# pjmikkol/bwtc

Hardware: AMD Instinct MI355X
Metric: MB/s compressed (BWT+encode) on 256 MiB block (higher is better)
Workload: dtype u8/u32/u64 integer

## Files before the change

### bwtc_amd/csrc/bwt_engine.hip

```cpp
#include "bwt_engine.hpp"
#include "radix_sort.hpp"
#include <algorithm>
#include <cmath>
#include <cstdlib>
#include <cstring>
#include <chrono>
#include <ctime>
#include <sys/prctl.h>

namespace bwtc_hip {

constexpr int kLoadTPB = 256;
constexpr int kLoadTile = kLoadTPB * 16;
constexpr u32 kTextPad = 128;

__global__ __launch_bounds__(kLoadTPB) void k_load_hist(const u8* __restrict__ src,
                                                        u8* __restrict__ T, u32 ncopy,
                                                        u32 padded, int reverse, int aligned,
                                                        u32* __restrict__ freqs) {
  __shared__ __attribute__((aligned(16))) u8 s_src[kLoadTile + 48];
  __shared__ u32 s_hist[256 * 16];
  const u32 tid = threadIdx.x;
  for (u32 i = tid; i < 256 * 16; i += kLoadTPB) s_hist[i] = 0;
  const u32 ntiles = (padded + (u32)kLoadTile - 1u) / (u32)kLoadTile;
// ... 1675 lines not shown
    if (std::getenv("BWTC_HIP_FIN_GROUP")) fin_max_group = std::atoi(std::getenv("BWTC_HIP_FIN_GROUP"));
    if (std::getenv("BWTC_HIP_FIN_WINDOW")) fin_window = std::atoi(std::getenv("BWTC_HIP_FIN_WINDOW"));
    fin_shape_fixed = std::getenv("BWTC_HIP_FIN_GROUP") || std::getenv("BWTC_HIP_FIN_WINDOW");
    fin_wide_short = !(std::getenv("BWTC_HIP_FIN_WIDE") && std::getenv("BWTC_HIP_FIN_WIDE")[0] == '0');
    fin_window = fin_window >= 2048 ? 2048 : 1024;
    fin_max_group = fin_max_group >= 1024 ? 1024 : fin_max_group >= 512 ? 512 : 256;
    if (fin_max_group >= fin_window) fin_max_group = fin_window / 2;
    code_keys = !(std::getenv("BWTC_HIP_KEYS") && std::strcmp(std::getenv("BWTC_HIP_KEYS"), "grams") == 0);
    if (std::getenv("BWTC_HIP_CODE_BITS")) code_bits = std::min(72, std::max(40, std::atoi(std::getenv("BWTC_HIP_CODE_BITS"))));
    finisher = !(std::getenv("BWTC_HIP_FINISHER") && std::getenv("BWTC_HIP_FINISHER")[0] == '0');
    gm_partition_lines = std::getenv("BWTC_HIP_GM_PARTITION") && std::strcmp(std::getenv("BWTC_HIP_GM_PARTITION"), "lines") == 0;
    wt_segmented = !(std::getenv("BWTC_HIP_SEG_STEPS") && std::getenv("BWTC_HIP_SEG_STEPS")[0] == '0');
    gram_min_n = kGramMinN;
    if (std::getenv("BWTC_HIP_GRAM_MIN_N")) gram_min_n = (u32)std::max(64, std::atoi(std::getenv("BWTC_HIP_GRAM_MIN_N")));
    if (std::getenv("BWTC_HIP_LONG_E")) long_items_per_thread = std::atoi(std::getenv("BWTC_HIP_LONG_E")) == 6 ? 6 : 8;
    if (std::getenv("BWTC_HIP_FIN_PASSES")) fin_max_passes = std::max(0, std::atoi(std::getenv("BWTC_HIP_FIN_PASSES")));
    if (std::getenv("BWTC_HIP_FIN_WORDS")) fin_words = std::min(4, std::max(2, std::atoi(std::getenv("BWTC_HIP_FIN_WORDS"))));
    if (std::getenv("BWTC_HIP_LONG_DIRECT")) long_direct = std::getenv("BWTC_HIP_LONG_DIRECT")[0] != '0';
    if (std::getenv("BWTC_HIP_FIN_ROUNDS")) fin_rounds = std::min(4, std::max(1, std::atoi(std::getenv("BWTC_HIP_FIN_ROUNDS"))));
    run_ranks = !(std::getenv("BWTC_HIP_RUNS") && std::getenv("BWTC_HIP_RUNS")[0] == '0');
    local_rounds = !(std::getenv("BWTC_HIP_LOCAL_ROUNDS") && std::getenv("BWTC_HIP_LOCAL_ROUNDS")[0] == '0');
    if (std::getenv("BWTC_HIP_FIN_FLOOR")) fin_floor = (u32)std::max(0, std::atoi(std::getenv("BWTC_HIP_FIN_FLOOR")));
    if (std::getenv("BWTC_HIP_TEXT_ROUNDS")) { text_rounds = std::max(0, std::atoi(std::getenv("BWTC_HIP_TEXT_ROUNDS"))); text_rounds_fixed = true; }
    const char* hg = std::getenv("BWTC_HIP_HUGE_MI");
    if (hg && std::atoi(hg) > 0) huge_group_elements = (u64)std::atoi(hg) << 20;
  }
  if (std::getenv("BWTC_HIP_SCAN") && std::strcmp(std::getenv("BWTC_HIP_SCAN"), "chained") == 0) {
    scan_chain.cap_tiles = (u32)(cap / kScanTile + 4096);
    BWTC_HIP_TRY(hipMalloc(reinterpret_cast<void**>(&scan_chain.status), ((u64)scan_chain.cap_tiles + 1) * 8));
    BWTC_HIP_TRY(hipMemset(scan_chain.status, 0, ((u64)scan_chain.cap_tiles + 1) * 8));
    scan_chain.ticket = scan_chain.status + scan_chain.cap_tiles;
    scan_chain.err = d_small + 522;
    scan_chain.stream = stream;
    scan_chain.issued = 0;
    scan_chain.epoch = 0;
  }
  BWTC_HIP_TRY(hipHostMalloc(reinterpret_cast<void**>(&h_small), 1024 * 4, hipHostMallocDefault));
  BWTC_HIP_TRY(hipHostMalloc(reinterpret_cast<void**>(&h_stage), cap + 32, hipHostMallocDefault));
  BWTC_HIP_TRY(hipEventCreateWithFlags(&ev_wait, hipEventBlockingSync | hipEventDisableTiming));
  {
    const char* m = std::getenv("BWTC_HIP_SYNC");
    wait_mode = m && std::strcmp(m, "spin") == 0 ? 1 : m && std::strcmp(m, "block") == 0 ? 2 : 0;
  }
  BWTC_HIP_TRY(hipEventCreate(&ev_begin));
  BWTC_HIP_TRY(hipEventCreate(&ev_end));
  for (int i = 0; i < kMaxSortEvents; ++i) BWTC_HIP_TRY(hipEventCreate(&ev_sort[i]));
// ... 530 lines not shown
        if (rc) return rc;
        w_bits = gp.b * lk.G2;
        if (w_bits < kRadixBits) { lk.first_r = w_bits; lk.first_mask = (1u << std::min(kRadixBits, w_bits + key_bits)) - 1u; }
        short_len = (u32)(gp.g * (gp.G + lk.G2));
        h = (u64)short_len;
        hipLaunchKernelGGL(k_make_keys_gram, dim3(ceil_div(n, 1024)), dim3(256), 0, st, d_T, d_lut,
                           (const uint4*)d_rank, ka, (u32*)nullptr, n, gp.g, gp.G, gp.b, plan.sigma, gp.top, key_plane, split, lk);
        lg.hi_shift = lk.hi_shift; lg.chr_shift = lk.chr_shift; lg.chr_mask = lk.chr_mask; lg.lvl_shift = -1; lg.depth = short_len;
        if (std::getenv("BWTC_HIP_DEBUG"))
          std::fprintf(stderr, "long keys: %d + %d bits, %d + %d grams of %d characters, character code at bit %d\n",
                       key_bits, w_bits, gp.G, lk.G2, gp.g, lk.chr_shift);
      }
    }
    if (lk.w) {
      u64* ks = nullptr; unsigned short* vs16 = nullptr; u32* ws = nullptr;
      u32* vs32 = nullptr;
      if (!split_now)
        radix_sort_long<u32, 6>(ka, kb, d_V0, d_V1, d_W0, d_W1, n, key_bits, w_bits, d_table, d_partial, stream, &ks, &vs32, &ws, &probe, d_P0, d_P1, 0, false, long_direct);
      else if (long_items_per_thread == 6)
        radix_sort_long<unsigned short, 6>(ka, kb, reinterpret_cast<unsigned short*>(d_V0), reinterpret_cast<unsigned short*>(d_V1),
                                           d_W0, d_W1, n, key_bits, w_bits, d_table, d_partial, stream, &ks, &vs16, &ws, &probe, d_P0, d_P1, 0, false, long_direct);
      else
        radix_sort_long<unsigned short, 8>(ka, kb, reinterpret_cast<unsigned short*>(d_V0), reinterpret_cast<unsigned short*>(d_V1),
                                           d_W0, d_W1, n, key_bits, w_bits, d_table, d_partial, stream, &ks, &vs16, &ws, &probe, d_P0, d_P1, 0, false, long_direct);
      BWTC_HIP_TRY(hipEventRecord(ev_sort[n_sort_events++], st));
      u32* vs = split_now ? reinterpret_cast<u32*>(vs16) : vs32;
      rb.rec_keys = ks; rb.rec_free = ks == ka ? kb : ka;
      rb.v_keys = vs; rb.v_free = vs == d_V0 ? d_V1 : d_V0;
      lg.w = ws; lg.wmask = w_bits >= 32 ? ~0u : (1u << w_bits) - 1u;
      rc = rank_step<u64, true>(ks, vs, n, n, short_len, (1ull << key_bits) - 1ull, rb, re, emit, h, &res, (u32)split_now, &lg);
      if (rc == -3 && coded && (h_small[kSmallError] & 2u)) {
        if (std::getenv("BWTC_HIP_DEBUG")) std::fprintf(stderr, "code keys: a codeword above %u bits, the block takes gram keys\n", kCodeMaxLen);
        BWTC_HIP_TRY(hipMemsetAsync(d_small + kSmallError, 0, 4, st));
        code_failed = true;
        rc = suffix_sort(n, hist, lone_sentinel, em);
        code_failed = false;
        return rc;
      }
      if (rc) return rc;
      const int long_passes = (key_bits + w_bits + kRadixBits - 1) / kRadixBits;
      stats.sort_pass_items += (u64)n * (u64)long_passes;
      stats.alg_bytes += (u64)n * (1 + 12 + 1)
                         + sort_bytes(n, long_passes, split_now ? 14 : 16, 8, true);
      stats.route |= coded ? 17u : 1u;
      key_bits = 0;
    } else if (gp.G > 0) {
      hipLaunchKernelGGL(k_make_keys_gram, dim3(ceil_div(n, 1024)), dim3(256), 0, st, d_T, d_lut,
// ... 549 lines not shown
```

### bwtc_amd/csrc/bwt_engine.hpp

```cpp
#pragma once
#include "common.hpp"
#include "bwtc_hip.h"
#include "radix_sort.hpp"
#include "scan.hpp"
#include "wavelet_host.hpp"
#include "wavelet_pipeline.hpp"
#include <sys/mman.h>
#include <condition_variable>
#include <future>
#include <map>
#include <mutex>
#include <thread>
#include <memory>
#include <utility>
#include <cstdlib>
#include <functional>
#include <vector>

namespace bwtc_hip {

struct RrEmit;
struct RrLong;
struct FinList;
struct FinShallow;
// ... 307 lines not shown
  int suffix_sort(u32 n, const u32* hist, bool lone_sentinel, const EmitTarget* em = nullptr);
  template <typename K>
  void sort_pairs(K* k0, K* k1, u32* v0, u32* v1, u64 n, int nbits, K** ks, u32** vs,
                  bool probe_it, int bit_lo = 0, u64 n_holes = 0, bool plane_ready = false, bool values_descend = false);
  struct RankBuffers { void* rec_keys; void* rec_free; u32* v_keys; u32* v_free; u32* aglob; u32* aglob_next; };
  struct RankResult { u32 m, groups; u64* ks; u32* vs; void* rec_other; u32* v_other; bool finish; u32 text_chars; bool carry;
                      bool ran_run; };
  template <typename K, bool INIT>
  int rank_step(const K* ks, const u32* vs, u32 m, u32 n, u32 short_len, K kmask, RankBuffers& rb,
                struct RrEmit re, bool emit, u64 h_next, RankResult* res, u32 split = 0,
                const struct RrLong* lg = nullptr, bool text = false, bool carry_in = true, bool raw_out = false,
                int run_mode = 0);
  bool dense_route = true;
  bool digit_planes = true;
  int window_bits = 16;
  bool split_index = true;
  bool gram_keys = true;
  int gram_count_override = 0;
  struct GramPlan { int g = 0, G = 0, b = 0; u32 top = 0; };
  int plan_grams(const KeyPlan& plan, u32 n, const u8* d_lut, GramPlan* gp);
  bool no_emit = false;
  bool long_keys = true;
  int long_items_per_thread = 8;
  u32 gram_min_n = 1u << 22;
  bool code_failed = false;
  bool code_keys = true;
  int code_bits = 72;
  u32* d_pairs = nullptr;
  u32* d_codes = nullptr;
  u32* d_parkS = nullptr;
  u64* d_parkHP = nullptr;
  u32 parked = 0;
  u32 park_holes = 0;
  u32* d_hardS = nullptr;
  u64* d_hardHP = nullptr;
  unsigned short* d_hardC = nullptr;
  bool ranks_live = false;
  u32 fin_floor = 12;
  bool finisher = true;
  int fin_window = 1024;
  int fin_max_group = 256;
  int fin_words = 2;
  bool fin_shape_fixed = false;
  bool fin_wide_short = true;
  int fin_window_blk = 1024;
  int fin_group_blk = 256;
// ... 72 lines not shown
```

### bwtc_amd/csrc/c_abi.hip

```cpp
#include "bwt_engine.hpp"
#include "gpu_lanes.hpp"
#include "huffman_decoder.hpp"
#include "postprocess.hpp"
#include "wavelet_rebuild.hpp"
#include "prepr_host.hpp"
#include <new>
#include "radix_sort.hpp"
#include "bwtc_hip.h"
#include "entropy_host.hpp"
#include "wavelet_host.hpp"
#include "wavelet_gpu_models.hpp"
#include <sched.h>
#include <algorithm>
#include <atomic>
#include <string>
#include <cstring>
#include <new>
#include <thread>
#include <vector>

using namespace bwtc_hip;

struct bwtc_hip_ctx {
  BwtEngine eng;
// ... 131 lines not shown
  V* v1 = reinterpret_cast<V*>(e.d_V1);
  std::vector<u8> plane(n);
  if (wbits >= kRadixBits) {
    for (u64 i = 0; i < n; ++i) plane[i] = (u8)(w[i] & 255u);
  } else {
    const u32 dmask = (1u << std::min(kRadixBits, wbits + kbits)) - 1u;
    for (u64 i = 0; i < n; ++i) plane[i] = (u8)((w[i] | ((u32)keys[i] << wbits)) & dmask);
  }
  SortCanaries can;
  BWTC_HIP_TRY(hipMemcpyAsync(k0, keys, n * 8, hipMemcpyHostToDevice, st));
  BWTC_HIP_TRY(hipMemcpyAsync(e.d_W0, w, n * 4, hipMemcpyHostToDevice, st));
  BWTC_HIP_TRY(hipMemcpyAsync(e.d_P0, plane.data(), n, hipMemcpyHostToDevice, st));
  BWTC_HIP_TRY(hipMemsetAsync(v0, 0xA5, n * sizeof(V), st));
  BWTC_HIP_TRY(can.put(k0, n * 8, st));
  BWTC_HIP_TRY(can.put(k1, n * 8, st));
  BWTC_HIP_TRY(can.put(v0, n * sizeof(V), st));
  BWTC_HIP_TRY(can.put(v1, n * sizeof(V), st));
  BWTC_HIP_TRY(can.put(e.d_W0, n * 4, st));
  BWTC_HIP_TRY(can.put(e.d_W1, n * 4, st));
  BWTC_HIP_TRY(can.put(e.d_P0, n, st));
  BWTC_HIP_TRY(can.put(e.d_P1, n, st));
  u64* ks = nullptr; V* vs = nullptr; u32* ws = nullptr;
  radix_sort_long<V, EL>(k0, k1, v0, v1, e.d_W0, e.d_W1, n, kbits, wbits, e.d_table, e.d_partial, st, &ks, &vs, &ws, nullptr,
                         e.d_P0, e.d_P1, 0, false, direct_w);
  BWTC_HIP_TRY(hipMemcpyAsync(keys, ks, n * 8, hipMemcpyDeviceToHost, st));
  BWTC_HIP_TRY(hipMemcpyAsync(vals, vs, n * sizeof(V), hipMemcpyDeviceToHost, st));
  BWTC_HIP_TRY(hipMemcpyAsync(w, ws, n * 4, hipMemcpyDeviceToHost, st));
  BWTC_HIP_TRY(can.fetch(st));
  BWTC_HIP_TRY(e.wait());
  BWTC_HIP_TRY(hipGetLastError());
  return can.verdict();
}
}

static std::mutex& host_allocs_mu() { static std::mutex m; return m; }
static std::map<void*, std::pair<int, uint64_t> >& host_allocs() { static std::map<void*, std::pair<int, uint64_t> > m; return m; }

static __global__ __launch_bounds__(256) void k_copy_probe(const uint4* __restrict__ src, uint4* __restrict__ dst, uint64_t n16) {
  const uint64_t i = (uint64_t)blockIdx.x * 256u + threadIdx.x;
  if (i < n16) dst[i] = src[i];
}

extern "C" {

int bwtc_hip_device_count(void) {
  int n = 0;
  if (hipGetDeviceCount(&n) != hipSuccess) return 0;
// ... 877 lines not shown

int bwtc_hip_test_radix_pairs(bwtc_hip_ctx* ctx, void* keys, void* vals, uint64_t n, uint64_t n_holes, int key_bytes, int val_bytes,
                              int bit_lo, int nbits, int values_mode, int planes) {
  if (!ctx || !keys) return -1;
  BwtEngine& e = ctx->eng;
  typedef unsigned short u16v;
  if (key_bytes == 4 && val_bytes == 4) return test_radix_pairs<u32, u32>(e, static_cast<u32*>(keys), static_cast<u32*>(vals), n, n_holes, bit_lo, nbits, values_mode, planes);
  if (key_bytes == 8 && val_bytes == 4) return test_radix_pairs<u64, u32>(e, static_cast<u64*>(keys), static_cast<u32*>(vals), n, n_holes, bit_lo, nbits, values_mode, planes);
  if (key_bytes == 4 && val_bytes == 2) return test_radix_pairs<u32, u16v>(e, static_cast<u32*>(keys), static_cast<u16v*>(vals), n, n_holes, bit_lo, nbits, values_mode, planes);
  if (key_bytes == 8 && val_bytes == 2) return test_radix_pairs<u64, u16v>(e, static_cast<u64*>(keys), static_cast<u16v*>(vals), n, n_holes, bit_lo, nbits, values_mode, planes);
  return -1;
}

int bwtc_hip_test_radix_long(bwtc_hip_ctx* ctx, uint64_t* keys, void* vals, uint32_t* w, uint64_t n, int val_bytes, int items_per_thread,
                             int kbits, int wbits, int direct_w) {
  if (!ctx || !keys || !vals || !w) return -1;
  BwtEngine& e = ctx->eng;
  typedef unsigned short u16v;
  if (val_bytes == 4 && items_per_thread == 6) return test_radix_long<u32, 6>(e, keys, static_cast<u32*>(vals), w, n, kbits, wbits, direct_w != 0);
  if (val_bytes == 2 && items_per_thread == 6) return test_radix_long<u16v, 6>(e, keys, static_cast<u16v*>(vals), w, n, kbits, wbits, direct_w != 0);
  if (val_bytes == 2 && items_per_thread == 8) return test_radix_long<u16v, 8>(e, keys, static_cast<u16v*>(vals), w, n, kbits, wbits, direct_w != 0);
  return -1;
}

int bwtc_hip_test_radix_segmented(bwtc_hip_ctx* ctx, uint32_t* keys, uint64_t n, int bit_lo, const uint32_t* tile_first, uint32_t nseg) {
  if (!ctx || !keys || !tile_first) return -1;
  BwtEngine& e = ctx->eng;
  const u64 tile = (u64)radix_tile<u32>();
  if (n == 0 || n % tile != 0 || n + kSortCanaryBytes > e.cap) return -1;
  if (bit_lo < 0 || bit_lo + 2 * kRadixBits > 32) return -1;
  if (nseg == 0 || (u64)nseg + 1 > e.cap || tile_first[0] != 0 || (u64)tile_first[nseg] != n / tile) return -1;
  for (u32 s = 0; s < nseg; ++s) if (tile_first[s] > tile_first[s + 1]) return -1;
  BWTC_HIP_TRY(hipSetDevice(e.device));
  hipStream_t st = e.stream;
  u32* k0 = static_cast<u32*>(e.d_R1);
  u32* k1 = static_cast<u32*>(e.d_R2);
  std::vector<u8> plane(n);
  for (u64 i = 0; i < n; ++i) plane[i] = (u8)((keys[i] >> bit_lo) & 255u);
  SortCanaries can;
  BWTC_HIP_TRY(hipMemcpyAsync(k0, keys, n * 4, hipMemcpyHostToDevice, st));
  BWTC_HIP_TRY(hipMemcpyAsync(e.d_P0, plane.data(), n, hipMemcpyHostToDevice, st));
  BWTC_HIP_TRY(hipMemcpyAsync(e.d_V0, tile_first, ((u64)nseg + 1) * 4, hipMemcpyHostToDevice, st));
  BWTC_HIP_TRY(can.put(k0, n * 4, st));
  BWTC_HIP_TRY(can.put(k1, n * 4, st));
  BWTC_HIP_TRY(can.put(e.d_P0, n, st));
  BWTC_HIP_TRY(can.put(e.d_P1, n, st));
// ... 217 lines not shown
```

### bwtc_amd/csrc/radix_sort.hpp

```cpp
#pragma once
#include "common.hpp"
#include "scan.hpp"
#include <algorithm>

namespace bwtc_hip {

constexpr int kRadixBits = 8;
constexpr int kRadixBins = 1 << kRadixBits;
#ifndef BWTC_RADIX_TPB
#define BWTC_RADIX_TPB 512
#endif
#ifndef BWTC_RADIX_E64
#define BWTC_RADIX_E64 8
#endif
#ifndef BWTC_RADIX_E32
#define BWTC_RADIX_E32 16
#endif
#ifndef BWTC_HIST_COPIES
#define BWTC_HIST_COPIES 16
#endif
constexpr int kRadixTPB = BWTC_RADIX_TPB;
constexpr int kRadixWaves = kRadixTPB / kWave;

#ifdef BWTC_RADIX_CHECKED
// ... 217 lines not shown
    kk[e] = i < tile_out ? s_key[i] : (K)0;
    vv[e] = (i < tile_out && !KEYS) ? s_val[i] : 0u;
    if (LONG) ww[LONG ? e : 0] = i < tile_out ? s_w[i] : 0u;
  }
#pragma unroll
  for (int e = 0; e < E; ++e)
    dst[e] = s_gofs[long_digit<K, LONG>(kk[e], ww[LONG ? e : 0], shift, la.dmask, la.bridge)] + tid + (u32)e * kRadixTPB;
#pragma unroll
  for (int e = 0; e < E; ++e) {
#ifdef BWTC_RADIX_CHECKED
    if (tid + (u32)e * kRadixTPB < tile_out && (u64)dst[e] >= n) { atomicOr(&g_radix_fault, 1u); continue; }
#endif
    if (tid + (u32)e * kRadixTPB < tile_out) {
      kout[dst[e]] = kk[e];
      if (!KEYS) vout[dst[e]] = (V)vv[e];
      if (LONG) la.wout[dst[e]] = ww[LONG ? e : 0];
      if (PLANE) {
        if (LONG) plane[dst[e]] = (u8)((la.nfrom_w == 2 ? (ww[LONG ? e : 0] >> la.nshift) | ((u32)kk[e] << la.nbridge)
                                         : la.nfrom_w ? ww[LONG ? e : 0] >> la.nshift : (u32)(kk[e] >> la.nshift)) & la.ndmask);
        else plane[dst[e]] = (u8)radix_digit(kk[e], shift + kRadixBits);
      }
    }
  }
}

template <typename K, int E_ = RadixCfg<K>::E, bool SEG = false>
__global__ __launch_bounds__(kRadixTPB) void k_radix_hist_plane(const u8* __restrict__ plane,
                                                                u32* __restrict__ table, u64 n,
                                                                u32 ntiles, SegArgs sa) {
  constexpr int E = E_;
  constexpr int HALF = kRadixTPB / 2;
  constexpr int B = 2 * E;
  static_assert(B == 8 || B == 12 || B % 16 == 0, "8-byte, 12-byte or whole 16-byte loads");
  constexpr u32 C = BWTC_HIST_COPIES;
  __shared__ __attribute__((aligned(16))) u32 hist[2][kRadixBins * C];
  {
    uint4* z = reinterpret_cast<uint4*>(&hist[0][0]);
    for (u32 i = threadIdx.x; i < 2u * kRadixBins * C / 4u; i += kRadixTPB) z[i] = make_uint4(0, 0, 0, 0);
  }
  __syncthreads();
  const u32 half = threadIdx.x / HALF, t = threadIdx.x % HALF;
  const u32 npairs = (ntiles + 1u) / 2u, per_xcd = (npairs + 7u) / 8u;
  const u32 pair = (blockIdx.x & 7u) * per_xcd + (blockIdx.x >> 3);
  const u32 tile = pair * 2u + half;
  if (pair < npairs && tile < ntiles) {
    const u64 base = (u64)tile * (kRadixTPB * E) + (u64)t * B;
// ... 167 lines not shown

static inline void radix_sort_keys_segmented(u32* k0, u32* k1, u64 n, int bit_lo, const u32* tile_first, u32 nseg,
                                             u32* table, u32* partial, hipStream_t st, u32** k_sorted,
                                             u8* plane0, u8* plane1) {
  constexpr int E = RadixCfg<u32>::E;
  const u32 ntiles = (u32)(n / radix_tile<u32>());
  const dim3 sgrid(((ntiles + 7u) / 8u) * 8u), hgrid(hist_plane_grid(ntiles)), tpb(kRadixTPB);
  SegArgs sa; sa.tile_first = tile_first; sa.nseg = nseg;
  hipLaunchKernelGGL((k_radix_hist_plane<u32, E, true>), hgrid, tpb, 0, st, (const u8*)plane0, table, n, ntiles, sa);
  exclusive_scan_u32(table, (u64)ntiles * kRadixBins, partial, st);
  hipLaunchKernelGGL((k_radix_scatter<u32, false, true, true, u32, 0, E, true>), sgrid, tpb, 0, st, (const u32*)k0, (const u32*)nullptr, k1,
                     (u32*)nullptr, (const u32*)table, n, bit_lo, ntiles, 2, plane1, LongArgs(), sa);
  hipLaunchKernelGGL((k_radix_hist_plane<u32, E, true>), hgrid, tpb, 0, st, (const u8*)plane1, table, n, ntiles, sa);
  exclusive_scan_u32(table, (u64)ntiles * kRadixBins, partial, st);
  hipLaunchKernelGGL((k_radix_scatter<u32, false, false, true, u32, 0, E, true>), sgrid, tpb, 0, st, (const u32*)k1, (const u32*)nullptr, k0,
                     (u32*)nullptr, (const u32*)table, n, bit_lo + kRadixBits, ntiles, 2, (u8*)nullptr, LongArgs(), sa);
  *k_sorted = k0;
}

template <typename V, int EL = 8>
static inline void radix_sort_long(u64* k0, u64* k1, V* v0, V* v1, u32* w0, u32* w1, u64 n, int kbits, int wbits,
                                   u32* table, u32* partial, hipStream_t st, u64** k_sorted, V** v_sorted,
                                   u32** w_sorted, ScatterProbe* probe, u8* plane0, u8* plane1, int wlo = 0,
                                   bool values_given = false, bool direct_w = true) {
  u64 *kin = k0, *kout = k1;
  V *vin = v0, *vout = v1;
  u32 *win = w0, *wout = w1;
  struct Pass { int from_w, shift; u32 dmask; int bridge; };
  Pass ps[24];
  int np = 0;
  int s = 0;
  for (; s + kRadixBits <= wbits; s += kRadixBits) ps[np++] = Pass{1, wlo + s, (1u << kRadixBits) - 1u, 0};
  int ks = 0;
  if (s < wbits) {
    const int r = wbits - s;
    ps[np++] = Pass{2, wlo + s, (1u << std::min(kRadixBits, r + kbits)) - 1u, r};
    ks = std::min(kbits, kRadixBits - r);
  }
  for (; ks < kbits; ks += kRadixBits) ps[np++] = Pass{0, ks, (1u << std::min(kRadixBits, kbits - ks)) - 1u, 0};
  if (n > 1) {
    const u32 ntiles = ceil_div(n, (u64)kRadixTPB * EL);
    const dim3 sgrid(((ntiles + 7u) / 8u) * 8u);
    for (int p = 0; p < np; ++p) {
      const bool from_words = direct_w && p > 0 && ps[p].from_w == 1 && ps[p].dmask == (1u << kRadixBits) - 1u;
      if (from_words) hipLaunchKernelGGL((k_radix_hist_words<EL>), dim3(hist_plane_grid(ntiles)), dim3(kRadixTPB), 0, st, (const u32*)win, table, n, ps[p].shift, ntiles);
      else hipLaunchKernelGGL((k_radix_hist_plane<u64, EL>), dim3(hist_plane_grid(ntiles)), dim3(kRadixTPB), 0, st, (const u8*)plane0, table, n, ntiles, SegArgs());
      exclusive_scan_u32(table, (u64)ntiles * kRadixBins, partial, st);
      const bool last = p + 1 == np;
      const bool no_plane = last || (direct_w && ps[p + 1].from_w == 1 && ps[p + 1].dmask == (1u << kRadixBits) - 1u);
      LongArgs la;
      la.win = win; la.wout = wout; la.dmask = ps[p].dmask; la.bridge = ps[p].bridge;
      la.nshift = last ? 0 : ps[p + 1].shift; la.nfrom_w = last ? 0 : ps[p + 1].from_w; la.ndmask = last ? 0u : ps[p + 1].dmask;
      la.nbridge = last ? 0 : ps[p + 1].bridge;
      const int vmode = (p == 0 && !values_given) ? 3 : 0;
      const bool timed = probe && probe->begin(st);
#define BWTC_SCATTER_L(P, L) hipLaunchKernelGGL((k_radix_scatter<u64, false, P, false, V, L, EL>), sgrid, dim3(kRadixTPB), 0, st, kin, vin, kout, vout, table, n, ps[p].shift, ntiles, vmode, no_plane ? (u8*)nullptr : plane1, la, SegArgs())
      if (ps[p].from_w == 2) { if (no_plane) BWTC_SCATTER_L(false, 3); else BWTC_SCATTER_L(true, 3); }
      else if (ps[p].from_w) { if (no_plane) BWTC_SCATTER_L(false, 2); else BWTC_SCATTER_L(true, 2); }
      else { if (no_plane) BWTC_SCATTER_L(false, 1); else BWTC_SCATTER_L(true, 1); }
#undef BWTC_SCATTER_L
      if (timed) probe->end(st, 2 * n * (sizeof(u64) + sizeof(V) + sizeof(u32)) + (no_plane ? 0 : n));
      { u8* tp = plane0; plane0 = plane1; plane1 = tp; }
      { u64* t = kin; kin = kout; kout = t; }
      { V* t = vin; vin = vout; vout = t; }
      { u32* t = win; win = wout; wout = t; }
    }
  }
  *k_sorted = kin; *v_sorted = vin; *w_sorted = win;
}


constexpr int kChains = 1;
constexpr int kSweepMaxPasses = 8;
constexpr u32 kStAgg = 1u << 30, kStIncl = 2u << 30, kStErr = 3u << 30, kStMask = (1u << 30) - 1u;
constexpr u32 kSweepSpinLimit = 1u << 22;

struct SweepWs {
  u32* hist_all;
  u32* bases;
  u32* tickets;
  u32* status;
  u32* error;
// ... 236 lines not shown
```

### bwtc_amd/hip.py

```python
import ctypes
import os

import numpy as np

_HERE = os.path.dirname(os.path.abspath(__file__))
LIB_PATH = os.environ.get("BWTC_HIP_LIB") or os.path.join(_HERE, "lib", "libbwtc_hip.so")

_vp = ctypes.c_void_p
_u32 = ctypes.c_uint32
_u64 = ctypes.c_uint64


class BwtcHipError(RuntimeError):
    def __init__(self, msg, code=None):
        super().__init__(msg)
        self.code = code


E_NO_CODE, E_SHAPE, E_PAST_RECORD, E_RUNS, E_CAPACITY, E_LENGTH = -10, -11, -12, -13, -14, -15


class HuffmanDecodeStats(ctypes.Structure):
    _fields_ = [("route", _u32), ("sections", _u32), ("streams", _u32), ("host_syncs", _u32),
                ("retries", _u32), ("max_code_len", _u32), ("runs", _u64), ("tiles", _u64), ("map_entries", _u64),
# ... 140 lines not shown
REJECT_FLAGS, REJECT_COUNT, REJECT_SCAN, REJECT_STATE, REJECT_TEST = 1, 2, 4, 8, 16


class KernelTimers(ctypes.Structure):
    _fields_ = [("scatter_launches", _u64), ("scatter_bytes", _u64), ("scatter_ms", ctypes.c_double)]


EXPORTS = [
    "bwtc_hip_huffman_decode", "bwtc_hip_huffman_decode_device", "bwtc_hip_huffman_decode_stats_get",
    "bwtc_hip_device_count", "bwtc_hip_version", "bwtc_hip_workspace_bytes", "bwtc_hip_create",
    "bwtc_hip_destroy", "bwtc_hip_stream", "bwtc_hip_get_stats", "bwtc_hip_set_profiling",
    "bwtc_hip_get_kernel_timers", "bwtc_hip_copy_probe", "bwtc_hip_test_gpu_lanes", "bwtc_hip_malloc", "bwtc_hip_free", "bwtc_hip_memcpy_to_device",
    "bwtc_hip_memcpy_to_host", "bwtc_hip_host_alloc", "bwtc_hip_host_free",
    "bwtc_hip_memcpy_to_device_async", "bwtc_hip_copy_wait", "bwtc_hip_wavelet_host_clock", "bwtc_hip_wavelet_host_progress", "bwtc_hip_wavelet_latency", "bwtc_hip_wavelet_routes", "bwtc_hip_host_staging_bytes", "bwtc_hip_host_usable_cpus", "bwtc_hip_n_lf", "bwtc_hip_bwt",
    "bwtc_hip_bwt_block", "bwtc_hip_bwt_block_device", "bwtc_hip_inverse_bwt_block",
    "bwtc_hip_inverse_bwt_block_device", "bwtc_hip_compress_bound",
    "bwtc_hip_huffman_encode_device", "bwtc_hip_huffman_encode", "bwtc_hip_transform_and_encode",
    "bwtc_hip_wavelet_section_stats", "bwtc_hip_transform_and_encode_wavelet", "bwtc_hip_wavelet_encode",
    "bwtc_hip_wavelet_encode_device", "bwtc_hip_wavelet_encode_device_begin", "bwtc_hip_wavelet_encode_end",
    "bwtc_hip_wavelet_encode_device_prepare", "bwtc_hip_wavelet_encode_queue",
    "bwtc_hip_wavelet_depth", "bwtc_hip_wavelet_set_depth", "bwtc_hip_numa_node", "bwtc_hip_host_cpu_slice", "bwtc_hip_set_worker_cpus", "bwtc_hip_wavelet_reset", "bwtc_hip_wavelet_start", "bwtc_hip_host_wavelet_sections", "bwtc_hip_host_wavelet_streams", "bwtc_hip_host_wavelet_streams_lanes", "bwtc_hip_host_huffman_lengths", "bwtc_hip_host_huffman_codes", "bwtc_hip_host_serialize_shape",
    "bwtc_hip_host_sections", "bwtc_hip_host_bwtblock_header", "bwtc_hip_synth", "bwtc_hip_suffix_array",
    "bwtc_hip_test_sort_u32", "bwtc_hip_test_sort_u64", "bwtc_hip_test_scan_u32",
    "bwtc_hip_test_radix_pairs", "bwtc_hip_test_radix_long", "bwtc_hip_test_radix_segmented",
    "bwtc_hip_wavelet_depth_needed", "bwtc_hip_grammar_create", "bwtc_hip_grammar_destroy", "bwtc_hip_grammar_rules", "bwtc_hip_grammar_special_symbols",
    "bwtc_hip_grammar_is_special", "bwtc_hip_grammar_write", "bwtc_hip_grammar_read", "bwtc_hip_pair_replace_device",
    "bwtc_hip_test_pair_stats", "bwtc_hip_precompress", "bwtc_hip_host_precompress", "bwtc_hip_postprocess",
    "bwtc_hip_postprocess_device", "bwtc_hip_postprocess_block", "bwtc_hip_postprocess_stats_get",
    "bwtc_hip_host_postprocess_tiles",
    "bwtc_hip_wavelet_decoder_create", "bwtc_hip_wavelet_decoder_destroy", "bwtc_hip_wavelet_decoder_reset",
    "bwtc_hip_wavelet_decode_bwt_host",
    "bwtc_hip_wavelet_decode_counts", "bwtc_hip_wavelet_decoder_forest", "bwtc_hip_wavelet_rebuild", "bwtc_hip_wavelet_rebuild_device",
    "bwtc_hip_host_wavelet_rebuild", "bwtc_hip_wavelet_decode_stats_get",
]

_lib = None


def load():
    global _lib
    if _lib is not None:
        return _lib
    if not os.path.exists(LIB_PATH):
        raise BwtcHipError(
            "%s not found: build it with `make -C bwtc_amd/csrc` (or __graft_entry__.build()); "
            "there is no CPU fallback" % LIB_PATH)
    L = ctypes.CDLL(LIB_PATH)
# ... 690 lines not shown
        n = keys.size - n_holes
        mode = self.RADIX_VALUES[values]
        if mode == 0:
            vals = np.array(vals, dtype=vtype, copy=True)
            assert vals.size == keys.size
        elif mode != 2:
            vals = np.zeros(max(n, 1), vtype)
        else:
            vals = None
        nbits = 8 * keys.itemsize if nbits is None else nbits
        _check(self.lib.bwtc_hip_test_radix_pairs(self.handle, _ptr(keys), None if vals is None else _ptr(vals), n, n_holes, keys.itemsize,
                                                  vtype.itemsize, bit_lo, nbits, mode, planes), "bwtc_hip_test_radix_pairs")
        return keys[:n], (None if vals is None else vals[:n])

    def test_radix_long(self, keys, w, kbits, wbits, vtype=np.uint32, items_per_thread=6, direct_w=True):
        keys = np.array(keys, dtype=np.uint64, copy=True)
        w = np.array(w, dtype=np.uint32, copy=True)
        assert keys.size == w.size
        vals = np.zeros(max(keys.size, 1), np.dtype(vtype))
        _check(self.lib.bwtc_hip_test_radix_long(self.handle, _ptr(keys), _ptr(vals), _ptr(w), keys.size, vals.itemsize, items_per_thread,
                                                 kbits, wbits, 1 if direct_w else 0), "bwtc_hip_test_radix_long")
        return keys, vals[:keys.size], w

    def test_radix_segmented(self, keys, bit_lo, tile_first):
        keys = np.array(keys, dtype=np.uint32, copy=True)
        tf = np.array(tile_first, dtype=np.uint32, copy=True)
        assert tf.size >= 2
        _check(self.lib.bwtc_hip_test_radix_segmented(self.handle, _ptr(keys), keys.size, bit_lo, _ptr(tf), tf.size - 1),
               "bwtc_hip_test_radix_segmented")
        return keys


def host_cpu_slice(numa_node, rank, ranks):
    L = load()
    buf = np.zeros(4096, np.uint32)
    n = L.bwtc_hip_host_cpu_slice(int(numa_node), int(rank), int(ranks), _ptr(buf), buf.size)
    if n < 0:
        raise BwtcHipError("bwtc_hip_host_cpu_slice failed with code %d" % n)
    return [int(c) for c in buf[:n]]


def host_staging_bytes():
    L = load()
    a, b = ctypes.c_uint64(0), ctypes.c_uint64(0)
    L.bwtc_hip_host_staging_bytes(ctypes.byref(a), ctypes.byref(b))
    return a.value, b.value
# ... 6 lines not shown
```

### include/bwtc_hip.h

```cpp
#ifndef BWTC_HIP_H
#define BWTC_HIP_H
#include <stddef.h>
#include <stdint.h>

#ifdef __cplusplus
extern "C" {
#endif

typedef struct bwtc_hip_ctx bwtc_hip_ctx;

typedef struct bwtc_hip_stats {
  uint32_t n;
  uint32_t rounds;
  uint64_t active_sum;
  uint64_t sort_pass_items;
  float    ms_total;
  float    ms_sort;
  uint32_t route;
  uint32_t finisher_entries;
  uint64_t alg_bytes;
} bwtc_hip_stats;

typedef struct bwtc_hip_kernel_timers {
  uint64_t scatter_launches;
// ... 161 lines not shown
                                  const uint8_t* run_sym, const uint32_t* run_start,
                                  const uint32_t* run_freqs, const uint32_t* dist_offset,
                                  const uint32_t* dist_len, const uint32_t* dist_cnt,
                                  uint32_t threads, char coder, uint32_t* state, uint8_t* out,
                                  uint64_t out_cap, uint64_t* out_bytes);

void     bwtc_hip_host_huffman_lengths(const uint64_t* freqs, uint8_t* clen);
void     bwtc_hip_host_huffman_codes(const uint8_t* clen, uint32_t* code);
uint32_t bwtc_hip_host_serialize_shape(const uint8_t* clen, uint8_t* out, uint32_t cap);
uint32_t bwtc_hip_host_sections(const uint32_t* freqs, uint32_t* section_len);
uint32_t bwtc_hip_host_bwtblock_header(const uint32_t* lf, uint32_t n_lf, uint8_t* out, uint32_t cap);

int bwtc_hip_synth(char kind, uint64_t seed, uint64_t size, uint8_t* out);

int bwtc_hip_suffix_array(bwtc_hip_ctx* ctx, const uint8_t* T, uint32_t length, uint32_t* sa);

int bwtc_hip_test_sort_u32(bwtc_hip_ctx* ctx, uint32_t* keys, uint32_t* vals, uint64_t n, int nbits);
int bwtc_hip_test_sort_u64(bwtc_hip_ctx* ctx, uint64_t* keys, uint32_t* vals, uint64_t n, int nbits);
int bwtc_hip_test_scan_u32(bwtc_hip_ctx* ctx, uint32_t* data, uint64_t n);
int bwtc_hip_test_radix_pairs(bwtc_hip_ctx* ctx, void* keys, void* vals, uint64_t n, uint64_t n_holes, int key_bytes, int val_bytes,
                              int bit_lo, int nbits, int values_mode, int planes);
int bwtc_hip_test_radix_long(bwtc_hip_ctx* ctx, uint64_t* keys, void* vals, uint32_t* w, uint64_t n, int val_bytes, int items_per_thread,
                             int kbits, int wbits, int direct_w);
int bwtc_hip_test_radix_segmented(bwtc_hip_ctx* ctx, uint32_t* keys, uint64_t n, int bit_lo, const uint32_t* tile_first, uint32_t nseg);
int bwtc_hip_test_gpu_lanes(bwtc_hip_ctx* ctx, const uint16_t* w, uint64_t n, const uint64_t* bounds, uint32_t k, int mode,
                            uint8_t* out, uint64_t out_cap, uint64_t* offsets);

typedef struct bwtc_hip_grammar bwtc_hip_grammar;
bwtc_hip_grammar* bwtc_hip_grammar_create(void);
void     bwtc_hip_grammar_destroy(bwtc_hip_grammar* g);
uint32_t bwtc_hip_grammar_rules(const bwtc_hip_grammar* g);
uint32_t bwtc_hip_grammar_special_symbols(const bwtc_hip_grammar* g);
int      bwtc_hip_grammar_is_special(const bwtc_hip_grammar* g, unsigned symbol);
int      bwtc_hip_grammar_write(const bwtc_hip_grammar* g, uint8_t* out, uint64_t cap, uint64_t* bytes);
int      bwtc_hip_grammar_read(bwtc_hip_grammar* g, const uint8_t* in, uint64_t n, uint64_t* consumed);
int      bwtc_hip_pair_replace_device(bwtc_hip_ctx* ctx, bwtc_hip_grammar* g, const uint8_t* d_src, uint64_t n,
                                      uint8_t* d_dst, uint64_t* n_out, uint32_t* replaced);
int      bwtc_hip_test_pair_stats(bwtc_hip_ctx* ctx, const uint8_t* d_src, uint64_t n, uint32_t* pair_cnt, uint32_t* byte_cnt);
int      bwtc_hip_precompress(bwtc_hip_ctx* ctx, bwtc_hip_grammar* g, const char* options, uint8_t* block, uint64_t n,
                              uint64_t* n_out);
int      bwtc_hip_host_precompress(bwtc_hip_grammar* g, const char* options, uint8_t* block, uint64_t n, uint64_t* n_out);
int      bwtc_hip_postprocess(const bwtc_hip_grammar* g, const uint8_t* data, uint64_t n, uint8_t* out, uint64_t cap,
                              uint64_t* n_out);
int      bwtc_hip_postprocess_device(bwtc_hip_ctx* ctx, const bwtc_hip_grammar* g, const uint8_t* d_data, uint64_t n,
                                     uint8_t* d_out, uint64_t cap, uint64_t* n_out);
int      bwtc_hip_postprocess_block(bwtc_hip_ctx* ctx, const bwtc_hip_grammar* g, const uint8_t* data, uint64_t n,
// ... 106 lines not shown
```

Measured before the change: 7298.

## Add persistent XCD-partitioned radix scatter kernel that prefetches the next tile

Adds a persistent scatter kernel for the long-key radix sort (u16 values, 8 items per thread). It launches a fixed grid of about two workgroups per CU, splits the tiles among the eight XCDs, and loads the keys and w words of the next tile while ranking and scattering the current one. This aims to hide global load latency and cut per-tile launch and scheduling overhead in the scatter passes. The cost is more registers (launch bounds of 4), a hand-managed LDS union, and a fixed grid size; setting BWTC_HIP_SCATTER=tiles restores the old path.

Result: slower. 7074 (-3.1%).

```diff
diff --git a/bwtc_amd/csrc/bwt_engine.hip b/bwtc_amd/csrc/bwt_engine.hip
--- a/bwtc_amd/csrc/bwt_engine.hip
+++ b/bwtc_amd/csrc/bwt_engine.hip
@@ -1721,6 +1721,12 @@
     local_rounds = !(std::getenv("BWTC_HIP_LOCAL_ROUNDS") && std::getenv("BWTC_HIP_LOCAL_ROUNDS")[0] == '0');
     if (std::getenv("BWTC_HIP_FIN_FLOOR")) fin_floor = (u32)std::max(0, std::atoi(std::getenv("BWTC_HIP_FIN_FLOOR")));
     if (std::getenv("BWTC_HIP_TEXT_ROUNDS")) { text_rounds = std::max(0, std::atoi(std::getenv("BWTC_HIP_TEXT_ROUNDS"))); text_rounds_fixed = true; }
+    if (!(std::getenv("BWTC_HIP_SCATTER") && std::strcmp(std::getenv("BWTC_HIP_SCATTER"), "tiles") == 0)) {
+      int cus = 0;
+      BWTC_HIP_TRY(hipDeviceGetAttribute(&cus, hipDeviceAttributeMultiprocessorCount, device));
+      scatter_wgs = 8u * (u32)std::max(1, 2 * cus / 8);
+      if (std::getenv("BWTC_HIP_SCATTER_WGS")) scatter_wgs = (u32)std::min(1 << 16, std::max(8, std::atoi(std::getenv("BWTC_HIP_SCATTER_WGS")))) & ~7u;
+    }
     const char* hg = std::getenv("BWTC_HIP_HUGE_MI");
     if (hg && std::atoi(hg) > 0) huge_group_elements = (u64)std::atoi(hg) << 20;
   }
@@ -2297,7 +2303,8 @@
                                            d_W0, d_W1, n, key_bits, w_bits, d_table, d_partial, stream, &ks, &vs16, &ws, &probe, d_P0, d_P1, 0, false, long_direct);
       else
         radix_sort_long<unsigned short, 8>(ka, kb, reinterpret_cast<unsigned short*>(d_V0), reinterpret_cast<unsigned short*>(d_V1),
-                                           d_W0, d_W1, n, key_bits, w_bits, d_table, d_partial, stream, &ks, &vs16, &ws, &probe, d_P0, d_P1, 0, false, long_direct);
+                                           d_W0, d_W1, n, key_bits, w_bits, d_table, d_partial, stream, &ks, &vs16, &ws, &probe, d_P0, d_P1, 0, false, long_direct,
+                                           scatter_wgs);
       BWTC_HIP_TRY(hipEventRecord(ev_sort[n_sort_events++], st));
       u32* vs = split_now ? reinterpret_cast<u32*>(vs16) : vs32;
       rb.rec_keys = ks; rb.rec_free = ks == ka ? kb : ka;
diff --git a/bwtc_amd/csrc/bwt_engine.hpp b/bwtc_amd/csrc/bwt_engine.hpp
--- a/bwtc_amd/csrc/bwt_engine.hpp
+++ b/bwtc_amd/csrc/bwt_engine.hpp
@@ -353,6 +353,7 @@
   bool no_emit = false;
   bool long_keys = true;
   int long_items_per_thread = 8;
+  u32 scatter_wgs = 0;
   u32 gram_min_n = 1u << 22;
   bool code_failed = false;
   bool code_keys = true;
diff --git a/bwtc_amd/csrc/c_abi.hip b/bwtc_amd/csrc/c_abi.hip
--- a/bwtc_amd/csrc/c_abi.hip
+++ b/bwtc_amd/csrc/c_abi.hip
@@ -177,7 +177,7 @@
   BWTC_HIP_TRY(can.put(e.d_P1, n, st));
   u64* ks = nullptr; V* vs = nullptr; u32* ws = nullptr;
   radix_sort_long<V, EL>(k0, k1, v0, v1, e.d_W0, e.d_W1, n, kbits, wbits, e.d_table, e.d_partial, st, &ks, &vs, &ws, nullptr,
-                         e.d_P0, e.d_P1, 0, false, direct_w);
+                         e.d_P0, e.d_P1, 0, false, direct_w, e.scatter_wgs);
   BWTC_HIP_TRY(hipMemcpyAsync(keys, ks, n * 8, hipMemcpyDeviceToHost, st));
   BWTC_HIP_TRY(hipMemcpyAsync(vals, vs, n * sizeof(V), hipMemcpyDeviceToHost, st));
   BWTC_HIP_TRY(hipMemcpyAsync(w, ws, n * 4, hipMemcpyDeviceToHost, st));
@@ -1101,6 +1101,8 @@
   if (val_bytes == 2 && items_per_thread == 8) return test_radix_long<u16v, 8>(e, keys, static_cast<u16v*>(vals), w, n, kbits, wbits, direct_w != 0);
   return -1;
 }
+
+uint32_t bwtc_hip_scatter_workgroups(bwtc_hip_ctx* ctx) { return ctx ? ctx->eng.scatter_wgs : 0u; }
 
 int bwtc_hip_test_radix_segmented(bwtc_hip_ctx* ctx, uint32_t* keys, uint64_t n, int bit_lo, const uint32_t* tile_first, uint32_t nseg) {
   if (!ctx || !keys || !tile_first) return -1;
diff --git a/bwtc_amd/csrc/radix_sort.hpp b/bwtc_amd/csrc/radix_sort.hpp
--- a/bwtc_amd/csrc/radix_sort.hpp
+++ b/bwtc_amd/csrc/radix_sort.hpp
@@ -263,6 +263,201 @@
       }
     }
   }
+}
+
+typedef unsigned short u16x2 __attribute__((ext_vector_type(2)));
+struct LongPipeLds {
+  u64* s_key; u32* s_w; unsigned short* s_val;
+  u32 (*s_cnt)[kRadixBins];
+  u32 *s_base, *s_gofs, *s_scr;
+};
+template <bool FULL, typename T, typename S>
+__device__ __forceinline__ void long_tile_load(T (&dst)[8], const S* __restrict__ src, u64 n, u32 tile, u32 wslot) {
+  constexpr int E = 8, TILE = kRadixTPB * E;
+  const u64 tile_base = (u64)tile * TILE;
+  const u64 left = n - tile_base;
+  const u32 tile_n = left < (u64)TILE ? (u32)left : (u32)TILE;
+#pragma unroll
+  for (int e = 0; e < E; ++e) {
+    const u32 slot = wslot + e * kWave;
+    dst[e] = (T)src[tile_base + (FULL ? slot : min(slot, tile_n - 1u))];
+  }
+}
+
+template <bool PLANE, int LONG, bool MADE, bool MORE>
+__device__ __forceinline__ void long_pipe_trip(
+    const LongPipeLds& L, u64 (&nk)[LONG != 2 ? 8 : 1], u32 (&nw)[LONG != 1 ? 8 : 1], u32 tile, u32 next,
+    const u64* __restrict__ kin, const unsigned short* __restrict__ vin, u64* __restrict__ kout,
+    unsigned short* __restrict__ vout, const u32* __restrict__ table, u64 n, int shift, u32 ntiles,
+    u8* __restrict__ plane, const LongArgs& la) {
+  typedef u64 K;
+  typedef unsigned short V;
+  constexpr int E = 8;
+  constexpr int TILE = kRadixTPB * E;
+  constexpr bool KEY_AHEAD = LONG != 2, W_AHEAD = LONG != 1;
+  u32 tid = threadIdx.x;
+  asm volatile("" : "+v"(tid));
+  const u32 wave = tid / kWave, lane = tid % kWave;
+  const u32 wslot = wave * (kWave * E) + lane;
+  const u64 tile_base = (u64)tile * TILE;
+  const u64 left = n - tile_base;
+  const u32 tile_n = MORE ? (u32)TILE : left < (u64)TILE ? (u32)left : (u32)TILE;
+  __syncthreads();
+  for (u32 i = tid; i < kRadixWaves * kRadixBins; i += kRadixTPB) (&L.s_cnt[0][0])[i] = 0;
+  K k[E];
+  u32 w[E];
+  u16x2 v[E / 2];
+  u32 r[E / 2];
+  if constexpr (KEY_AHEAD) {
+#pragma unroll
+    for (int e = 0; e < E; ++e) k[e] = nk[e];
+  }
+  if constexpr (W_AHEAD) {
+#pragma unroll
+    for (int e = 0; e < E; ++e) w[e] = nw[e];
+  }
+  if constexpr (!KEY_AHEAD) long_tile_load<MORE>(k, kin, n, tile, wslot);
+  if constexpr (!W_AHEAD) long_tile_load<MORE>(w, la.win, n, tile, wslot);
+#pragma unroll
+  for (int e = 0; e < E; ++e) {
+    const u32 slot = wslot + e * kWave;
+    if (MADE) v[e >> 1][e & 1] = (V)((u32)n - 1u - ((u32)tile_base + slot));
+    else if (MORE) v[e >> 1][e & 1] = vin[tile_base + slot];
+    else v[e >> 1][e & 1] = slot < tile_n ? vin[tile_base + slot] : (V)0;
+  }
+  const u32 tab = table[(u64)(tid & (kRadixBins - 1)) * ntiles + tile];
+  if constexpr (MORE) {
+    if constexpr (KEY_AHEAD) long_tile_load<false>(nk, kin, n, next, wslot);
+    if constexpr (W_AHEAD) long_tile_load<false>(nw, la.win, n, next, wslot);
+  }
+  __builtin_amdgcn_sched_barrier(0);
+  __syncthreads();
+
+#define BWTC_EXISTS(e) (MORE || (wslot + (e) * kWave) < tile_n)
+  volatile lds_u32* my_cnt = lds_volatile(&L.s_cnt[wave][0]);
+#pragma unroll
+  for (int e = 0; e < E; ++e) {
+    const bool ok = BWTC_EXISTS(e);
+    const u32 d = long_digit<K, LONG>(k[e], w[e], shift, la.dmask, la.bridge);
+    u32 below, peers;
+    wave_digit_rank<kRadixBits>(d, ok, &below, &peers);
+    u32 prev = 0;
+    if (ok) prev = my_cnt[d];
+    __builtin_amdgcn_wave_barrier();
+    if (e & 1) r[e >> 1] |= (prev + below) << 16;
+    else r[e >> 1] = prev + below;
+    if (ok && below + 1u == peers) my_cnt[d] = prev + peers;
+    __builtin_amdgcn_wave_barrier();
+  }
+  __syncthreads();
+
+  u32 dig_total = 0;
+  if (tid < kRadixBins) {
+#pragma unroll
+    for (int wv = 0; wv < kRadixWaves; ++wv) {
+      u32 c = L.s_cnt[wv][tid];
+      L.s_cnt[wv][tid] = dig_total;
+      dig_total += c;
+    }
+  }
+  u32 tile_valid;
+  u32 dig_base = block_scan_excl_add<kRadixTPB>(tid < kRadixBins ? dig_total : 0u, L.s_scr, &tile_valid);
+  if (tid < kRadixBins) {
+    L.s_base[tid] = dig_base;
+    L.s_gofs[tid] = tab - dig_base;
+  }
+  __syncthreads();
+
+#pragma unroll
+  for (int e = 0; e < E; ++e) {
+    if (BWTC_EXISTS(e)) {
+      const u32 d = long_digit<K, LONG>(k[e], w[e], shift, la.dmask, la.bridge);
+      r[e >> 1] += (L.s_base[d] + L.s_cnt[wave][d]) << (16 * (e & 1));
+    }
+  }
+  __syncthreads();
+#pragma unroll
+  for (int e = 0; e < E; ++e) {
+    if (BWTC_EXISTS(e)) {
+      const u32 slot = (r[e >> 1] >> (16 * (e & 1))) & 0xFFFFu;
+      L.s_key[slot] = k[e];
+      L.s_val[slot] = v[e >> 1][e & 1];
+      L.s_w[slot] = w[e];
+    }
+  }
+#undef BWTC_EXISTS
+  __syncthreads();
+
+  K kk[E];
+  u32 vv[E], dst[E], ww[E];
+#pragma unroll
+  for (int e = 0; e < E; ++e) {
+    const u32 i = tid + (u32)e * kRadixTPB;
+    kk[e] = (MORE || i < tile_n) ? L.s_key[i] : (K)0;
+    vv[e] = (MORE || i < tile_n) ? L.s_val[i] : 0u;
+    ww[e] = (MORE || i < tile_n) ? L.s_w[i] : 0u;
+  }
+#pragma unroll
+  for (int e = 0; e < E; ++e)
+    dst[e] = L.s_gofs[long_digit<K, LONG>(kk[e], ww[e], shift, la.dmask, la.bridge)] + tid + (u32)e * kRadixTPB;
+#pragma unroll
+  for (int e = 0; e < E; ++e) {
+#ifdef BWTC_RADIX_CHECKED
+    if ((MORE || tid + (u32)e * kRadixTPB < tile_n) && (u64)dst[e] >= n) { atomicOr(&g_radix_fault, 1u); continue; }
+#endif
+    if (MORE || tid + (u32)e * kRadixTPB < tile_n) {
+      kout[dst[e]] = kk[e];
+      vout[dst[e]] = (V)vv[e];
+      la.wout[dst[e]] = ww[e];
+      if (PLANE) plane[dst[e]] = (u8)((la.nfrom_w == 2 ? (ww[e] >> la.nshift) | ((u32)kk[e] << la.nbridge)
+                                       : la.nfrom_w ? ww[e] >> la.nshift : (u32)(kk[e] >> la.nshift)) & la.ndmask);
+    }
+  }
+}
+
+template <bool PLANE, int LONG, bool MADE>
+__global__ __launch_bounds__(kRadixTPB, 4) void k_radix_scatter_pipe(
+    const u64* __restrict__ kin, const unsigned short* __restrict__ vin, u64* __restrict__ kout,
+    unsigned short* __restrict__ vout, const u32* __restrict__ table, u64 n, int shift, u32 ntiles,
+    u8* __restrict__ plane, LongArgs la) {
+  static_assert(LONG >= 1 && LONG <= 3, "long items only");
+  constexpr int E = 8;
+  constexpr int TILE = kRadixTPB * E;
+  constexpr int kStageBytes = TILE * (int)(sizeof(u64) + sizeof(unsigned short) + sizeof(u32));
+  constexpr int kCntBytes = kRadixWaves * kRadixBins * (int)sizeof(u32);
+  __shared__ __attribute__((aligned(16))) unsigned char s_raw[kStageBytes > kCntBytes ? kStageBytes : kCntBytes];
+  __shared__ u32 s_base[kRadixBins];
+  __shared__ u32 s_gofs[kRadixBins];
+  __shared__ u32 s_scr[kRadixTPB / kWave + 1];
+  LongPipeLds L;
+  L.s_key = reinterpret_cast<u64*>(s_raw);
+  L.s_w = reinterpret_cast<u32*>(s_raw + TILE * sizeof(u64));
+  L.s_val = reinterpret_cast<unsigned short*>(s_raw + TILE * (sizeof(u64) + sizeof(u32)));
+  L.s_cnt = reinterpret_cast<u32 (*)[kRadixBins]>(s_raw);
+  L.s_base = s_base; L.s_gofs = s_gofs; L.s_scr = s_scr;
+
+  const u32 wslot = (threadIdx.x / kWave) * (kWave * E) + threadIdx.x % kWave;
+  const u32 per_xcd = (ntiles + 7u) / 8u, stride = gridDim.x >> 3;
+  const u32 xcd = blockIdx.x & 7u;
+  const u32 list_end = min((xcd + 1u) * per_xcd, ntiles);
+  u32 tile = xcd * per_xcd + (blockIdx.x >> 3);
+  if (tile >= list_end) return;
+
+  u64 nk[LONG != 2 ? E : 1];
+  u32 nw[LONG != 1 ? E : 1];
+  if constexpr (LONG != 2) long_tile_load<false>(nk, kin, n, tile, wslot);
+  if constexpr (LONG != 1) long_tile_load<false>(nw, la.win, n, tile, wslot);
+#define BWTC_TRIP(MORE) long_pipe_trip<PLANE, LONG, MADE, MORE>(L, nk, nw, tile, tile + stride, kin, vin, kout, vout, table, n, shift, ntiles, plane, la)
+  if (tile + stride < list_end) {
+    BWTC_TRIP(true);
+    tile += stride;
+    while (tile + stride < list_end) {
+      BWTC_TRIP(true);
+      tile += stride;
+    }
+  }
+  BWTC_TRIP(false);
+#undef BWTC_TRIP
 }
 
 template <typename K, int E_ = RadixCfg<K>::E, bool SEG = false>
@@ -476,7 +671,7 @@
 static inline void radix_sort_long(u64* k0, u64* k1, V* v0, V* v1, u32* w0, u32* w1, u64 n, int kbits, int wbits,
                                    u32* table, u32* partial, hipStream_t st, u64** k_sorted, V** v_sorted,
                                    u32** w_sorted, ScatterProbe* probe, u8* plane0, u8* plane1, int wlo = 0,
-                                   bool values_given = false, bool direct_w = true) {
+                                   bool values_given = false, bool direct_w = true, u32 pipe_wgs = 0) {
   u64 *kin = k0, *kout = k1;
   V *vin = v0, *vout = v1;
   u32 *win = w0, *wout = w1;
@@ -509,9 +704,24 @@
       const int vmode = (p == 0 && !values_given) ? 3 : 0;
       const bool timed = probe && probe->begin(st);
 #define BWTC_SCATTER_L(P, L) hipLaunchKernelGGL((k_radix_scatter<u64, false, P, false, V, L, EL>), sgrid, dim3(kRadixTPB), 0, st, kin, vin, kout, vout, table, n, ps[p].shift, ntiles, vmode, no_plane ? (u8*)nullptr : plane1, la, SegArgs())
-      if (ps[p].from_w == 2) { if (no_plane) BWTC_SCATTER_L(false, 3); else BWTC_SCATTER_L(true, 3); }
-      else if (ps[p].from_w) { if (no_plane) BWTC_SCATTER_L(false, 2); else BWTC_SCATTER_L(true, 2); }
-      else { if (no_plane) BWTC_SCATTER_L(false, 1); else BWTC_SCATTER_L(true, 1); }
+      const bool piped = sizeof(V) == 2 && EL == 8 && pipe_wgs >= 8u;
+      if constexpr (sizeof(V) == 2 && EL == 8) {
+        if (piped) {
+          const dim3 pgrid(std::min(pipe_wgs & ~7u, (u32)sgrid.x));
+#define BWTC_SCATTER_P(P, L) do { if (vmode) BWTC_SCATTER_PM(P, L, true); else BWTC_SCATTER_PM(P, L, false); } while (0)
+#define BWTC_SCATTER_PM(P, L, M) hipLaunchKernelGGL((k_radix_scatter_pipe<P, L, M>), pgrid, dim3(kRadixTPB), 0, st, kin, vin, kout, vout, table, n, ps[p].shift, ntiles, no_plane ? (u8*)nullptr : plane1, la)
+          if (ps[p].from_w == 2) { if (no_plane) BWTC_SCATTER_P(false, 3); else BWTC_SCATTER_P(true, 3); }
+          else if (ps[p].from_w) { if (no_plane) BWTC_SCATTER_P(false, 2); else BWTC_SCATTER_P(true, 2); }
+          else { if (no_plane) BWTC_SCATTER_P(false, 1); else BWTC_SCATTER_P(true, 1); }
+#undef BWTC_SCATTER_P
+#undef BWTC_SCATTER_PM
+        }
+      }
+      if (!piped) {
+        if (ps[p].from_w == 2) { if (no_plane) BWTC_SCATTER_L(false, 3); else BWTC_SCATTER_L(true, 3); }
+        else if (ps[p].from_w) { if (no_plane) BWTC_SCATTER_L(false, 2); else BWTC_SCATTER_L(true, 2); }
+        else { if (no_plane) BWTC_SCATTER_L(false, 1); else BWTC_SCATTER_L(true, 1); }
+      }
 #undef BWTC_SCATTER_L
       if (timed) probe->end(st, 2 * n * (sizeof(u64) + sizeof(V) + sizeof(u32)) + (no_plane ? 0 : n));
       { u8* tp = plane0; plane0 = plane1; plane1 = tp; }
diff --git a/bwtc_amd/hip.py b/bwtc_amd/hip.py
--- a/bwtc_amd/hip.py
+++ b/bwtc_amd/hip.py
@@ -186,7 +186,7 @@
     "bwtc_hip_wavelet_depth", "bwtc_hip_wavelet_set_depth", "bwtc_hip_numa_node", "bwtc_hip_host_cpu_slice", "bwtc_hip_set_worker_cpus", "bwtc_hip_wavelet_reset", "bwtc_hip_wavelet_start", "bwtc_hip_host_wavelet_sections", "bwtc_hip_host_wavelet_streams", "bwtc_hip_host_wavelet_streams_lanes", "bwtc_hip_host_huffman_lengths", "bwtc_hip_host_huffman_codes", "bwtc_hip_host_serialize_shape",
     "bwtc_hip_host_sections", "bwtc_hip_host_bwtblock_header", "bwtc_hip_synth", "bwtc_hip_suffix_array",
     "bwtc_hip_test_sort_u32", "bwtc_hip_test_sort_u64", "bwtc_hip_test_scan_u32",
-    "bwtc_hip_test_radix_pairs", "bwtc_hip_test_radix_long", "bwtc_hip_test_radix_segmented",
+    "bwtc_hip_test_radix_pairs", "bwtc_hip_test_radix_long", "bwtc_hip_test_radix_segmented", "bwtc_hip_scatter_workgroups",
     "bwtc_hip_wavelet_depth_needed", "bwtc_hip_grammar_create", "bwtc_hip_grammar_destroy", "bwtc_hip_grammar_rules", "bwtc_hip_grammar_special_symbols",
     "bwtc_hip_grammar_is_special", "bwtc_hip_grammar_write", "bwtc_hip_grammar_read", "bwtc_hip_pair_replace_device",
     "bwtc_hip_test_pair_stats", "bwtc_hip_precompress", "bwtc_hip_host_precompress", "bwtc_hip_postprocess",
@@ -923,6 +923,11 @@
                                                  kbits, wbits, 1 if direct_w else 0), "bwtc_hip_test_radix_long")
         return keys, vals[:keys.size], w
 
+    def scatter_workgroups(self):
+        f = self.lib.bwtc_hip_scatter_workgroups
+        f.restype, f.argtypes = _u32, [_vp]
+        return int(f(self.handle))
+
     def test_radix_segmented(self, keys, bit_lo, tile_first):
         keys = np.array(keys, dtype=np.uint32, copy=True)
         tf = np.array(tile_first, dtype=np.uint32, copy=True)
diff --git a/include/bwtc_hip.h b/include/bwtc_hip.h
--- a/include/bwtc_hip.h
+++ b/include/bwtc_hip.h
@@ -207,6 +207,7 @@
                               int bit_lo, int nbits, int values_mode, int planes);
 int bwtc_hip_test_radix_long(bwtc_hip_ctx* ctx, uint64_t* keys, void* vals, uint32_t* w, uint64_t n, int val_bytes, int items_per_thread,
                              int kbits, int wbits, int direct_w);
+uint32_t bwtc_hip_scatter_workgroups(bwtc_hip_ctx* ctx);
 int bwtc_hip_test_radix_segmented(bwtc_hip_ctx* ctx, uint32_t* keys, uint64_t n, int bit_lo, const uint32_t* tile_first, uint32_t nseg);
 int bwtc_hip_test_gpu_lanes(bwtc_hip_ctx* ctx, const uint16_t* w, uint64_t n, const uint64_t* bounds, uint32_t k, int mode,
                             uint8_t* out, uint64_t out_cap, uint64_t* offsets);
```
